# moabarar/nemar

Measured on AMD Instinct MI355X. Metric: train images/sec (256x256 A/B pairs), higher is better.
Workload: dtype f32

## Files before the change

include/nemar_hip.h:

```cpp
#ifndef NEMAR_HIP_H
#define NEMAR_HIP_H
#include <stddef.h>

#ifdef __cplusplus
extern "C" {
#endif

#define NEMAR_OK 0
#define NEMAR_EINVAL (-1)
#define NEMAR_ELAUNCH (-2)
#define NEMAR_EWORKSPACE (-3)

int nemar_version(void);
const char* nemar_last_error(void);

#define NEMAR_GRID_EXPLICIT 0
#define NEMAR_GRID_UNET 1
#define NEMAR_GRID_AFFINE 2
int nemar_grid_sample_fwd(const float* in, const float* grid_src, int grid_mode, float* out,
                          int N, int C, int H, int W, int Ho, int Wo, void* stream);
size_t nemar_grid_sample_bwd_workspace(int N, int C, int H, int W);
size_t nemar_grid_sample_bwd_zeroed_bytes(int N, int C, int H, int W);
int nemar_grid_sample_bwd(const float* in, const float* grid_src, int grid_mode, const float* gout,
                          float* gin, int accum_gin, float* ggrid, int accum_ggrid,
// ... 63 lines not shown
int nemar_conv2d_bwd_weight_ex(const float* x0, int C0, const float* x1, int C1, const float* gy, float* gw, float* gb, int N,
                               int H, int W, int K, int OH, int OW, int R, int S, int stride, int pad, int pad_mode,
                               void* workspace, size_t ws_bytes, void* stream, const nemar_conv_extras* extras);
int nemar_pack_plan_record(int plan);
int nemar_pack_plan_jobs(int plan);
size_t nemar_pack_plan_bytes(int plan);
int nemar_pack_plan_dirty(int plan);
int nemar_pack_plan_commit(int plan, void* device_buffer, size_t bytes, void* stream);
int nemar_pack_plan_run(int plan, void* stream);
int nemar_pack_plan_reset(int plan);
int nemar_last_route(void);
int nemar_config_epoch(void);
int nemar_set_max_words_lazy(int on);
int nemar_max_words_finalize(void* max_words, int samples, void* stream);
size_t nemar_conv2d_scratch(int N, int H, int W, int K, int C, int R, int S, int stride, int pad);
int nemar_absmax(const float* t, long long n, void* out_word, void* stream);
int nemar_absmax_samples(const float* t, int samples, long long per_sample, void* out_words, void* stream);
int nemar_kernel_timer(int enable);
int nemar_kernel_timer_read(double* total_ms, double* total_flop, int* launches);
size_t nemar_bias_grad_workspace(int N, int C, int HW);
int nemar_bias_grad(const float* g, float* gb, int N, int C, int HW, void* workspace, size_t ws_bytes, void* stream);

int nemar_instnorm_fwd(const float* x, const float* residual, float* y, float* stats, int planes, int HW,
                       float eps, int act, float slope, void* stream);
int nemar_instnorm_bwd(const float* x, const float* stats, const float* gy, float* gx, int planes, int HW,
                       int act, float slope, void* stream);
#define NEMAR_MAX_PARTIALS 2048
#define NEMAR_MAX_WORDS(samples) ((size_t)(samples) * (1 + NEMAR_MAX_PARTIALS))
int nemar_instnorm_fwd_max(const float* x, const float* residual, float* y, float* stats, int planes, int HW,
                           float eps, int act, float slope, void* max_words, int planes_per_sample, void* stream);
// ... 99 lines not shown
```

nemar_amd/_lib.py:

```python
import ctypes as C
import os

import torch

_HERE = os.path.dirname(os.path.abspath(__file__))
PRODUCT_PATH = os.path.join(_HERE, "lib", "libnemar_hip.so")
AB_PATH = os.path.join(_HERE, "lib", "libnemar_hip_ab.so")
DEFAULT_PATH = AB_PATH if (os.environ.get("NEMAR_AB_LIBRARY") == "1" or os.environ.get("NEMAR_TUNE")) else PRODUCT_PATH

_f = C.POINTER(C.c_float)
_vp = C.c_void_p
_i = C.c_int
_fl = C.c_float
_sz = C.c_size_t
_ll = C.c_longlong
_db = C.c_double
_u64 = C.c_ulonglong
_u32 = C.c_uint

SIGNATURES = {
    "nemar_version": (_i, []),
    "nemar_last_error": (C.c_char_p, []),
    "nemar_grid_sample_fwd": (_i, [_vp, _vp, _i, _vp, _i, _i, _i, _i, _i, _i, _vp]),
    "nemar_grid_sample_bwd_workspace": (_sz, [_i, _i, _i, _i]),
# ... 2 lines not shown
    "nemar_smoothness_workspace": (_sz, [_i, _i, _i]),
    "nemar_smoothness_fwd": (_i, [_vp, _vp, _i, _fl, _fl, _vp, _i, _vp, _sz, _i, _i, _i, _vp]),
    "nemar_smoothness_bwd": (_i, [_vp, _vp, _i, _fl, _vp, _fl, _vp, _i, _i, _i, _i, _vp]),
    "nemar_fold_penalty_workspace": (_sz, [_i, _i, _i]),
    "nemar_fold_penalty_fwd": (_i, [_vp, _fl, _fl, _vp, _i, _vp, _vp, _sz, _i, _i, _i, _vp]),
    "nemar_fold_penalty_bwd": (_i, [_vp, _fl, _vp, _fl, _vp, _i, _i, _i, _i, _vp]),
    "nemar_conv2d_fwd_workspace": (_sz, [_i] * 9),
    "nemar_conv2d_fwd": (_i, [_vp, _i, _vp, _i, _vp, _vp, _vp, _i, _i, _i, _i, _i, _i, _i, _i, _i, _i, _fl, _vp, _sz, _i, _vp]),
    "nemar_conv2d_bwd_data_workspace": (_sz, [_i] * 10),
    "nemar_conv2d_bwd_data": (_i, [_vp, _vp, _vp, _i, _fl, _vp, _i, _vp, _i, _i, _i, _i, _i, _i, _i, _i, _i, _i, _i,
                                   _i, _vp, _sz, _i, _vp]),
    "nemar_conv2d_bwd_weight_workspace": (_sz, [_i] * 11),
    "nemar_conv2d_bwd_weight": (_i, [_vp, _i, _vp, _i, _vp, _vp, _vp, _i, _i, _i, _i, _i, _i, _i, _i, _i, _i, _i, _vp, _sz,
                                     _vp]),
    "nemar_conv2d_scratch": (_sz, [_i] * 9),
    "nemar_conv2d_gy_planes_bytes": (_sz, [_i] * 10),
    "nemar_absmax": (_i, [_vp, _ll, _vp, _vp]),
    "nemar_absmax_samples": (_i, [_vp, _i, _ll, _vp, _vp]),
    "nemar_kernel_timer": (_i, [_i]),
    "nemar_kernel_timer_read": (_i, [C.POINTER(C.c_double), C.POINTER(C.c_double), C.POINTER(_i)]),
    "nemar_bias_grad_workspace": (_sz, [_i, _i, _i]),
    "nemar_bias_grad": (_i, [_vp, _vp, _i, _i, _i, _vp, _sz, _vp]),
    "nemar_last_route": (_i, []),
    "nemar_last_gy_planes": (_i, []),
    "nemar_config_epoch": (_i, []),
    "nemar_set_max_words_lazy": (_i, [_i]),
    "nemar_instnorm_fwd": (_i, [_vp, _vp, _vp, _vp, _i, _i, _fl, _i, _fl, _vp]),
    "nemar_instnorm_bwd": (_i, [_vp, _vp, _vp, _vp, _i, _i, _i, _fl, _vp]),
    "nemar_instnorm_fwd_max": (_i, [_vp, _vp, _vp, _vp, _i, _i, _fl, _i, _fl, _vp, _i, _vp]),
    "nemar_instnorm_fwd_planes": (_i, [_vp, _vp, _vp, _vp, _vp, _i, _i, _i, _i, _fl, _i, _fl, _fl, _u64, _u32, _vp, _vp, _vp, _vp, _vp]),
# ... 159 lines not shown
```

nemar_amd/csrc/conv.hip:

```cpp
#define NEMAR_CONV_HIP
#include "common.h"
#include "conv_exact.h"
#include "conv_call.h"
#include "conv_route.h"
#include "pack_plan.h"

#ifdef NEMAR_AB
extern int g_split16_ring3;
extern int g_split16_ksplit_cap;
extern int g_narrow_fwd4;
extern int g_wg_xreg;
extern int g_register_vec4;
extern int g_overlap_per_lane;
extern int g_histogram_per_lane;
void nemar_norm_planes_debug(int bits);
#endif

int nemar_narrow_fwd(const float* x, const float* w, const float* bias, float* y, int N, int C, int H, int W, int K, int R,
                     int pad, int border, int act, float slope, float* part, size_t part_floats, hipStream_t st);
int nemar_narrow_wgrad(const float* x, const float* gy, float* gw, int N, int C, int H, int W, int K, int R, int pad,
                       int border, float* part, hipStream_t st);
void nemar_wgrad2_launch(const float* x0, int C0, const float* x1, int C1, const float* gy, float* gw, float* gb, int N,
                         int H, int W, int K, int OH, int OW, int R, int S, int stride, int pad, int pad_mode,
                         int target_blocks, bool vec_ok, int dbg, float* part, hipStream_t st);
// ... 796 lines not shown
        if (gb) bias_grad_slabs(gy, gb, part ? part + P.bias_off : nullptr, N, K, OH * OW, st);
        what = "conv2d_bwd_weight (narrow)";
        break;
    case WgradPlan::S16G:
        nemar_s16g_wgrad(x0, C0, x1, C1, gy, gw, gb, N, H, W, K, OH, OW, R, stride, pad_mode, part, g_dbg, st);
        what = "conv2d_bwd_weight (16-bit pipe, in-kernel split)";
        break;
    case WgradPlan::SPLIT16:
        call.bias_rode = gb && call.bias_partials;
        nemar_split16_wgrad(x0, gy, gw, N, C0, H, W, K, R, pad_mode == BORDER_REFLECT ? 1 : 0, call.scratch, part, g_xcd_map,
                            R == 3 ? call.src2_planes : nullptr, (R == 3 && pad_mode == BORDER_REFLECT) ? call.x_planes : nullptr,
                            call.src_max, call.src2_max, call.bias_rode ? call.bias_partials : nullptr, gb, st);
        if (gb && !call.bias_rode) bias_grad_slabs(gy, gb, part + P.bias_off, N, K, OH * OW, st);
        what = "conv2d_bwd_weight (split-16)";
        break;
    case WgradPlan::WGRAD2:
        nemar_wgrad2_launch(x0, C0, x1, C1, gy, gw, gb, N, H, W, K, OH, OW, R, S, stride, pad, pad_mode, g_wgrad_blocks,
                            g_wgrad != 2, g_dbg, part, st);
        what = "conv2d_bwd_weight (wide)";
        break;
    case WgradPlan::WGRAD2_PADDED_GY: {
        float* gyp = part + P.gyp_off;
        const long long total = (long long)N * K * P.ohv * OW;
        hipLaunchKernelGGL(pad_planes_kernel, dim3(nemar_stream_grid(total, 256)), dim3(256), 0, st, gy, gyp, OH * OW, P.ohv * OW, total);
        nemar_wgrad2_launch(x0, C0, x1, C1, gyp, gw, gb, N, H, W, K, P.ohv, OW, R, S, stride, pad, pad_mode, g_wgrad_blocks,
                            g_wgrad != 2, g_dbg, part, st);
        what = "conv2d_bwd_weight (wide, padded gy)";
        break;
    }
    case WgradPlan::LEGACY: {
// ... 25 lines not shown
NEMAR_API int nemar_tune_ptr(void* p) { g_tl = (long long*)p; return NEMAR_OK; }

NEMAR_API int nemar_tune(int key, int value) {
    ++g_config_epoch;
    if (key == 0) { g_cfg128 = value; return NEMAR_OK; }
    if (key == 1) { g_lds_pad = value; return NEMAR_OK; }
    if (key == 2) { g_dbg = value; return NEMAR_OK; }
    if (key == 3) { g_narrow = value; return NEMAR_OK; }
    if (key == 4) { g_wgrad = value; return NEMAR_OK; }
    if (key == 6) { g_min_blocks = value > 0 ? value : 384; return NEMAR_OK; }
    if (key == 14) { g_deterministic = value != 0; return NEMAR_OK; }
    if (key == 8) { g_reflect_aux = value != 0; return NEMAR_OK; }
    if (key == 15) { g_xcd_map = value != 0; return NEMAR_OK; }
    if (key == 20) { g_split16 = value != 0; return NEMAR_OK; }
    if (key == 24) { g_s16g = value != 0; return NEMAR_OK; }
    if (key == 25) { g_s16g_min_mmac = value < 0 ? 0 : value; return NEMAR_OK; }
    if (key == 26) { g_s16g_wgrad_first = value != 0; return NEMAR_OK; }
    if (key == 27) { nemar_s16g_tune(0, value); return NEMAR_OK; }
    if (key == 29) { g_s16g_wgrad = value != 0; return NEMAR_OK; }
    if (key == 31) { nemar_norm_planes_debug(value); return NEMAR_OK; }
    if (key == 32) { g_split16_ring3 = value != 0; return NEMAR_OK; }
    if (key == 33) { g_k7 = value != 0; return NEMAR_OK; }
    if (key == 36) { g_split_act = value != 0; return NEMAR_OK; }
    if (key == 43) { g_fold_small = value != 0; return NEMAR_OK; }
    if (key == 37) { g_lds_claim = value; return NEMAR_OK; }
    if (key == 38) { g_wg_xreg = value != 0; return NEMAR_OK; }
    if (key == 39) { g_split16_ksplit_cap = value < 1 ? 1 : (value > 8 ? 8 : value); return NEMAR_OK; }
    if (key == 45) { g_overlap_per_lane = value != 0; return NEMAR_OK; }
    if (key == 46) { g_histogram_per_lane = value != 0; return NEMAR_OK; }
    if (key == 44) { g_register_vec4 = value != 0; return NEMAR_OK; }
// ... 20 lines not shown
}
#endif

static DgradPlan usual_dgrad(int N, int C, int H, int W, int K, int R, int S, int stride, int pad, int pad_mode) {
    DgradPlan P{};
    if (N <= 0 || C <= 0 || H <= 0 || W <= 0 || K <= 0 || R <= 0 || S <= 0 || stride < 1) return P;
    return plan_dgrad({N, C, 0, H, W, K, R, S, stride, pad, pad_mode}, ConvFacts::canonical());
}
static bool fusable(const DgradPlan& P) { return P.gy_planes_need != 0 && P.split16_ksplit == 1; }

NEMAR_API size_t nemar_conv2d_scratch(int N, int H, int W, int K, int C, int R, int S, int stride, int pad) {
    if (N <= 0 || H <= 0 || W <= 0 || K <= 0 || C <= 0) return 0;
    return plan_arena_bytes({N, C, 0, H, W, K, R, S, stride, pad, BORDER_ZERO});
}

NEMAR_API size_t nemar_conv2d_gy_planes_bytes(int N, int C, int H, int W, int K, int R, int S, int stride, int pad, int pad_mode) {
    return usual_dgrad(N, C, H, W, K, R, S, stride, pad, pad_mode).gy_planes_need;
}

NEMAR_API int nemar_conv2d_bwd_data_fusable(int N, int C, int H, int W, int K, int R, int S, int stride, int pad, int pad_mode) {
    return fusable(usual_dgrad(N, C, H, W, K, R, S, stride, pad, pad_mode)) ? 1 : 0;
}

NEMAR_API int nemar_conv2d_bwd_data_addend_ok(int N, int C, int H, int W, int K, int R, int S, int stride, int pad, int pad_mode) {
    const DgradPlan P = usual_dgrad(N, C, H, W, K, R, S, stride, pad, pad_mode);
    if (fusable(P)) return 1;
    if (pad_mode != BORDER_REFLECT || pad <= 0 || stride != 1 || pad >= H || pad >= W || R != S || R == 7) return 0;
    return (P.fold16 || P.fold) && plan_arena_bytes({N, C, 0, H, W, K, R, S, stride, pad, BORDER_ZERO}) == 0 ? 1 : 0;
}

// ... 128 lines not shown
```

nemar_amd/csrc/conv_route.h:

```cpp
#pragma once
#ifndef NEMAR_CONV_HIP
#error "conv_route.h holds conv.hip's own switches: include it from conv.hip only"
#endif
#include "common.h"
#include "conv_exact.h"
#include "conv_split16.h"
#include "conv_s16g.h"
#include "conv_k7.h"

bool nemar_narrow_eligible(int K, int C1, int R, int S, int stride, int N, int OH, int OW);
int nemar_narrow_wgrad_splits(int N, int C, int OH, int OW);
bool nemar_wgrad2_eligible(int K, int OH, int OW, bool gy_aligned16);
void nemar_wgrad2_plan(int K, int J, int P, int target_blocks, int* splits_out, int* pix_per_split_out);

using namespace nemar_exact;

namespace {

static NEMAR_SWITCH(int, g_split16, 1);
static NEMAR_SWITCH(long long, g_split16_min_mmac, 2000);
static NEMAR_SWITCH(int, g_split16_variant, 4);
static NEMAR_SWITCH(int, g_k7, 1);
static NEMAR_SWITCH(int, g_s16g, 1);
static NEMAR_SWITCH(long long, g_s16g_min_mmac, 30);
static NEMAR_SWITCH(int, g_s16g_wgrad, 1);
static NEMAR_SWITCH(int, g_s16g_wgrad_first, 0);
static NEMAR_SWITCH(int, g_s16g_fold, 1);
static NEMAR_SWITCH(int, g_split_act, 1);
static NEMAR_SWITCH(int, g_fold_small, 1);
static NEMAR_SWITCH(int, g_dual_gy, 1);
static NEMAR_SWITCH(int, g_reflect_aux, 1);
static NEMAR_SWITCH(int, g_deterministic, 1);
static NEMAR_SWITCH(int, g_ksplit, 1);
static NEMAR_SWITCH(int, g_narrow, 1);
static NEMAR_SWITCH(int, g_wgrad, 0);
static NEMAR_SWITCH(int, g_wgrad_blocks, 512);

// ... 308 lines not shown
        L.route = ROUTE_S16G; L.sub = DgradPlan::S16G;
        L.q.act = f.act; L.q.slope = f.slope;
    } else if (L.fold16 && f.gx0 && !f.gx1 && !f.bias && f.act == ACT_NONE) {
        L.route = ROUTE_S16G; L.sub = DgradPlan::S16G_FOLD;
    } else {
        L.route = ROUTE_EXACT; L.sub = DgradPlan::EXACT;
        L.narrow = g_narrow && stride == 1 && !L.fold && !f.bias && f.act == ACT_NONE && L.mskip == 0 && !f.gx1 && R - 1 - pad >= 0 &&
                   nemar_narrow_eligible(C, 0, R, S, 1, N, H, W);
        L.split = !L.narrow && L.ksplit > 1 && !f.bias && f.act == ACT_NONE && L.mskip == 0 &&
                  (L.fold ? (f.gx0 && !f.gx1) : (!f.gx1 || (f.gx0 && !L.ring)));
        L.aux_rows = !L.narrow && L.ring && g_reflect_aux && pad == 1 && R == 3 && S == 3 && H >= 4 && W >= 8;
    }
    return L;
}

void legacy_wgrad_plan(int K, int J, int P, int* splits_out, int* pix_per_split_out) {
    const bool wide = K > 32;
    const int BM = wide ? 128 : 32, BN = wide ? 128 : 256;
    const int mt = nemar_cdiv(K, BM), jt = nemar_cdiv(J, BN);
    int splits = nemar_cdiv(1024, mt * jt);
    const int max_splits = nemar_cdiv(P, WBK * 8);
    if (splits > max_splits) splits = max_splits;
    if (splits < 1) splits = 1;
    if (splits > 65535) splits = 65535;
    *pix_per_split_out = nemar_cdiv(nemar_cdiv(P, splits), WBK) * WBK;
    *splits_out = nemar_cdiv(P, *pix_per_split_out);
}
int padded_rows(int OH, int OW) {
    int ohv = OH;
    while ((ohv * OW) % 4) ++ohv;
    return ohv;
}
bool wgrad_pad_route(int K, int OH, int OW, int pad_mode) {
    return K > 4 && (OH * OW) % 4 != 0 && pad_mode == BORDER_ZERO && g_wgrad != 1;
}

struct WgradPlan {
    int route;
    enum Sub { K7, NARROW, S16G, SPLIT16, WGRAD2, WGRAD2_PADDED_GY, LEGACY } sub;
    size_t total, bias_off, gyp_off;
    int splits, pix_per_split, ohv;
};
WgradPlan plan_wgrad(const ConvShape& s, const ConvFacts& f) {
    WgradPlan P;
    const int N = s.N, C = s.C(), H = s.H, W = s.W, K = s.K, R = s.R, S = s.S, stride = s.stride, pad = s.pad, OH = s.OH(), OW = s.OW();
    const int J = C * R * S, Pix = N * OH * OW, ohv = padded_rows(OH, OW);
    const size_t slab = (size_t)K * J, bias_parts = (size_t)N * nemar_cdiv(OH * OW, BIAS_CHUNK) * K;
    int w2_splits, legacy_splits, pad_splits = 0, pps;
    nemar_wgrad2_plan(K, J, Pix, g_wgrad_blocks, &w2_splits, &pps);
    legacy_wgrad_plan(K, J, Pix, &legacy_splits, &P.pix_per_split);
    P.total = (size_t)(w2_splits > legacy_splits ? w2_splits : legacy_splits) * (slab + K);
    if ((OH * OW) % 4 != 0 && K > 4) {
        nemar_wgrad2_plan(K, J, N * ohv * OW, g_wgrad_blocks, &pad_splits, &pps);
        grow(P.total, (size_t)pad_splits * (slab + K) + 4 + (size_t)N * K * ohv * OW);
    }
    if (K <= 4) grow(P.total, (size_t)nemar_narrow_wgrad_splits(N, C, OH, OW) * slab + bias_parts);
    if (nemar_s16g_wgrad_eligible(N, C, 0, H, W, K, OH, OW, R, S, stride, pad, BORDER_ZERO))
        grow(P.total, (size_t)nemar_s16g_wgrad_slabs_max(N, C, K, OH, W, stride) * (slab + K));
    const bool k7 = nemar_k7_wgrad_eligible(N, C, H, W, K, R, S, stride, pad);
    if (k7) grow(P.total, nemar_k7_wgrad_floats(N, C, H, W, K) + bias_parts);
    const bool wide = wide_candidates(s).wgrad;
    if (wide) grow(P.total, (size_t)nemar_split16_wgrad_splits(N, C, H, W, K, R) * slab + bias_parts);
    const bool s16g_wg = g_s16g_wgrad && f.part && s16g_worth_it(s.macs()) &&
                         nemar_s16g_wgrad_eligible(N, s.C0, s.C1, H, W, K, OH, OW, R, S, stride, pad, s.pad_mode);
    const bool split16_wg = g_split16 && g_split16_variant == 4 && f.part && s.C1 == 0 && split16_worth_it(N, OH, OW, K, C, R, S) && wide &&
                            (R == 3 || s.pad_mode == BORDER_ZERO) && f.scratch_bytes &&
                            f.scratch_bytes >= nemar_split16_wgrad_scratch_bytes(N, C, H, W, K, R);
    P.bias_off = P.gyp_off = 0; P.splits = 0; P.ohv = ohv;
    if (g_k7 && f.part && s.C1 == 0 && k7) {
        P.route = ROUTE_K7; P.sub = WgradPlan::K7; P.bias_off = nemar_k7_wgrad_floats(N, C, H, W, K);
    } else if (nemar_narrow_eligible(K, s.C1, R, S, stride, N, OH, OW) && g_narrow) {
        P.route = ROUTE_NARROW; P.sub = WgradPlan::NARROW; P.bias_off = (size_t)nemar_narrow_wgrad_splits(N, s.C0, OH, OW) * slab;
    } else if (s16g_wg && (g_s16g_wgrad_first || !split16_wg)) {
        P.route = ROUTE_S16G; P.sub = WgradPlan::S16G;
    } else if (split16_wg) {
        P.route = ROUTE_SPLIT16; P.sub = WgradPlan::SPLIT16; P.bias_off = (size_t)nemar_split16_wgrad_splits(N, C, H, W, K, R) * slab;
    } else {
        P.route = ROUTE_EXACT;
        P.gyp_off = ((size_t)pad_splits * (slab + K) + 3) & ~(size_t)3;
        const bool padded_gy = f.part && wgrad_pad_route(K, OH, OW, s.pad_mode) && nemar_wgrad2_eligible(K, ohv, OW, f.part_aligned);
        if (g_wgrad != 1 && nemar_wgrad2_eligible(K, OH, OW, f.gy_aligned)) P.sub = WgradPlan::WGRAD2;
        else if (padded_gy) P.sub = WgradPlan::WGRAD2_PADDED_GY;
        else { P.sub = WgradPlan::LEGACY; P.splits = legacy_splits; P.bias_off = (size_t)legacy_splits * slab; }
    }
    return P;
}

size_t plan_arena_bytes(const ConvShape& s) {
    const int N = s.N, C = s.C(), H = s.H, W = s.W, K = s.K, R = s.R;
    if (!g_split16 || !split16_worth_it(N, H + 2 * s.pad - R + 1, W + 2 * s.pad - s.S + 1, K, C, R, s.S)) return 0;
    const WideCandidates c = wide_candidates(s);
    size_t b = c.fwd ? nemar_split16_scratch_total(N, H, W, K, C, H, W) : 0;
    if (c.dgrad) grow(b, nemar_split16_scratch_total(N, H, W, C, K, H, W));
    if (c.wgrad) grow(b, nemar_split16_wgrad_scratch_bytes(N, C, H, W, K, R));
    return b;
}

}
```

nemar_amd/csrc/conv_split16.h:

```cpp
#pragma once
#include <hip/hip_runtime.h>
#include <stddef.h>
#include "conv_call.h"

enum { SPLIT16_ZERO = 0, SPLIT16_REFLECT = 1, SPLIT16_DGRAD_REFLECT = 2 };

bool nemar_split16_eligible(int N, int H, int W, int M, int Cred, int R, int S, int stride, int pad, int mode, int variant);
size_t nemar_split16_scratch_bytes(int N, int Cred, int H, int W);
int nemar_split16_ksplit(int N, int H, int W, int M, int Cred);
size_t nemar_split16_scratch_total(int N, int H, int W, int M, int Cred, int OH, int OW);
size_t nemar_split16_pack_bytes(int M, int Cred, int KS);
void nemar_split16_pack(const float* w, void* packed, int K, int C, int KS, int dgrad, int variant, hipStream_t st);
struct Split16Done {
    bool dual_written;
    bool epilogue_fused;
};
Split16Done nemar_split16_conv(const float* src, const void* packed, const float* bias, float* dst, int N, int H, int W, int M, int Cred,
                               int KS, int src_pad, int Hs, int Ws_src, int OH, int OW, int mode, void* scratch, int xcd_map, int variant,
                               long long* tl, void* dual_g_out, MaxWords src_max, const void* ready_planes, int ready_kind,
                               const float* addend, void* out_max, hipStream_t st);

bool nemar_split16_wgrad_eligible(int N, int C, int H, int W, int K, int R, int S, int stride, int pad);
size_t nemar_split16_wgrad_scratch_bytes(int N, int C, int H, int W, int K, int KS);
int nemar_split16_wgrad_splits(int N, int C, int H, int W, int K, int KS);
#ifdef NEMAR_AB
void nemar_split16_wgrad_tune(int one_copy);
#endif
void nemar_sum_partials_pair(const float* part_a, long long stride_a, int splits_a, float* dst_a, long long n_a,
                             const float* part_b, long long stride_b, int splits_b, float* dst_b, long long n_b, bool accumulate, hipStream_t st);
void nemar_split16_wgrad(const float* x, const float* gy, float* gw, int N, int C, int H, int W, int K, int KS, int reflect,
                         void* scratch, float* part, int xcd_map, const void* g_planes, const void* x_planes, MaxWords x_max,
                         MaxWords gy_max, const float* bias_partials, float* gb, hipStream_t st);
size_t nemar_split16_wgrad_g_bytes(int N, int H, int W, int K, int KS);
void nemar_split16_dual_split(const float* gy, void* dplanes, void* gplanes, int N, int K, int H, int W, int mode, const unsigned* maxbits,
                              int mstride, hipStream_t st);
void nemar_sum_partials(const float* part, long long stride, int splits, float* dst, long long n, bool accumulate, hipStream_t st);
void nemar_sum_partials_two(const float* part, long long stride, int splits, float* d0, float* d1, int N, int C0, int C1, int HW, hipStream_t st);
void nemar_sum_partials_act(const float* part, long long stride, int splits, float* dst, long long n, int act, float slope, hipStream_t st);

void nemar_split16_absmax(const float* x, int samples, long long per, void* out, hipStream_t st);
const unsigned* nemar_split16_source_max(const float* src, int N, long long per, MaxWords hint, unsigned* own, int* stride, hipStream_t st);

void nemar_split16_timer(int on);
int nemar_split16_timer_read(double* total_ms, double* total_flop);
```

nemar_amd/csrc/conv_split16_wgrad.hip:

```cpp
#include "common.h"
#include "conv_split16.h"

namespace {

typedef float f32x16 __attribute__((ext_vector_type(16)));
typedef _Float16 f16x8 __attribute__((ext_vector_type(8)));
typedef unsigned u32x4 __attribute__((ext_vector_type(4)));

__device__ __forceinline__ float pow2_scale(unsigned maxbits) {
    const int e = (int)((maxbits >> 23) & 255u);
    if (e == 0 || e == 255) return 1.f;
    const int se = 127 + 11 - (e - 127);
    if (se < 1 || se > 254) return 1.f;
    return __builtin_bit_cast(float, (unsigned)se << 23);
}
__device__ __forceinline__ unsigned short f16_rn(float v) {
    const _Float16 h = (_Float16)v;
    return __builtin_bit_cast(unsigned short, h);
}
__device__ __forceinline__ void split2_f16(float v, unsigned short& h, unsigned short& l) {
    h = f16_rn(v);
    const float r = v - (float)__builtin_bit_cast(_Float16, h);
    l = f16_rn(r);
}
// ... 73 lines not shown
#pragma unroll
        for (int e = 0; e < 8; ++e) {
            const int xs = q * 8 + e - 1;
            v[e] = tile[cc][min(max(reflect ? mirror(xs, W) : xs, 0), W - 1)];
        }
#pragma unroll
        for (int e = 0; e < 8; ++e) {
            const int xp = q * 8 + e;
            const bool ok = xp < W + 2 && (reflect || (unsigned)(xp - 1) < (unsigned)W);
            split2_f16(ok ? v[e] : 0.f, h[e], l[e]);
        }
        const size_t t = (((size_t)n * CBLK + cblk) * FX + (size_t)yp * CPR + q) * 64 + cc;
        out[t] = pack8(h);
        out[total + t] = pack8(l);
    }
}

template <int TW>
__global__ __launch_bounds__(256) void split_dual_kernel(const float* __restrict__ gy, u32x4* __restrict__ dpl, u32x4* __restrict__ gpl,
                                                         int N, int K, int H, int W, int Hg, int CPR, int reflect, long long dtotal,
                                                         long long gtotal, const unsigned* maxbits, int mstride) {
    __shared__ float tile[64][TW + 1];
    const int Hp = H + 4, Ws = W + 4, KBLK = K >> 6, CG = K >> 3, F = Hg * CPR;
    const int prow = blockIdx.x % Hp, kblk = (blockIdx.x / Hp) % KBLK, n = blockIdx.x / (Hp * KBLK);
    const float scale = pow2_scale(maxbits[n * mstride]);
    const bool img = prow >= 1 && prow <= H;
    int ya = 0, yb = -1;
    bool any = img;
    if (img) ya = prow - 1;
    else if (reflect && prow == H + 2) { ya = 0; yb = 2; any = true; }
// ... 46 lines not shown
    const u32x4* G;
    const u32x4* X;
    float* part;
    int N, H, W, C, K;
    int CPR, F, FX, RB, spi;
    int KBLK, CBLK;
    long long gplane16, xplane16;
    const unsigned* gmax;
    const unsigned* xmax;
    int gstride, xstride;
    int xcd;
};

template <int KS, bool ONEG, bool XREG = false>
__global__ __launch_bounds__(256) void wgrad_split16_kernel(WgParams p) {
    static_assert(!XREG || (KS == 3 && ONEG), "XREG: instantiated and measured for the 3x3 one-copy form only");

    constexpr int GC = ONEG ? 1 : KS;
    constexpr int RING = 4, NCOL = 4 * GC + 4 * KS, NCP = NCOL / 4;
    constexpr int STAGE16 = NCOL * 64;
    constexpr int NMF = 3 * KS * KS, NSL = 2 * GC + 2 * KS + NCP;
    constexpr int NPV = KS / 2;
#ifdef NEMAR_HOST_EMULATION
    __shared__ __attribute__((aligned(16))) u32x4 smem[RING * STAGE16];
#else
    extern __shared__ __attribute__((aligned(16))) u32x4 smem[];
#endif
    const int tid = threadIdx.x, wid = __builtin_amdgcn_readfirstlane(tid >> 6), lane = tid & 63;
    const int tiles = p.KBLK * p.CBLK;
    int t = blockIdx.x;
    if (p.xcd) t = (t & 7) * ((int)gridDim.x >> 3) + (t >> 3);
// ... 280 lines not shown
    p.KBLK = KBLK; p.CBLK = CBLK;
    p.gplane16 = gtotal; p.xplane16 = xtotal;
    p.gmax = gmax; p.xmax = xmax; p.gstride = gstride; p.xstride = xstride;
    const int splits = N * p.spi, grid = splits * KBLK * CBLK;
    p.xcd = (xcd_map && grid % 8 == 0 && (grid / 8) % (KBLK * CBLK) == 0) ? 1 : 0;
    NEMAR_AB_ONLY(if (KS == 3 && oneg && !g_wg_xreg) wg_launch<3, true, false>(grid, p, st); else)
    if (KS == 3 && oneg) wg_launch<3, true, true>(grid, p, st);
    else if (oneg) wg_launch<4, true>(grid, p, st);
#ifdef NEMAR_AB
    else if (KS == 3) wg_launch<3, false>(grid, p, st);
    else wg_launch<4, false>(grid, p, st);
#endif
    nemar_sum_partials_pair(part, (long long)K * C * KS * KS, splits, gw, (long long)K * C * KS * KS, bias_partials, K, N,
                            bias_partials ? gb : nullptr, K, true, st);
}
```

nemar_amd/ops.py:

```python
import ctypes
import os
import weakref

import numpy as np

import torch
from torch.autograd import Function
from torch.autograd.function import once_differentiable

from . import _lib

L = _lib.load()



class _SizeQueries:

    def __init__(self, lib):
        self._lib, self._memo = lib, {}

    def __getattr__(self, name):
        fn = getattr(self._lib, name)
        memo = self._memo

# ... 185 lines not shown

def _conv_scratch(N, H, W, K, C, R, S, stride, pad, device):
    key = (N, H, W, K, C, R, S, stride, pad)
    need = _scratch_need.get(key)
    if need is None:
        need = _scratch_need[key] = L.conv2d_scratch(N, H, W, K, C, R, S, stride, pad)
    if not need:
        return None
    akey = (device, _lane[0])
    buf = _arena.get(akey)
    if buf is None or buf.numel() * 4 < need:
        _retire(buf)
        buf = torch.empty(int(need) // 4 + 64, dtype=torch.float32, device=device)
        _arena[akey] = buf
    return buf


_garena = {}
_garena_next = {}
_gplanes_need = {}
GY_RING = int(os.environ.get("NEMAR_GY_RING", "4"))
_GY_HANDOVER = os.environ.get("NEMAR_GY_HANDOVER", "1") == "1"


def _gy_planes(N, C, H, W, K, R, S, stride, pad, pad_mode, device):
    if _side_on[0] and not _GY_HANDOVER:
        return None, None
    key = (N, C, H, W, K, R, S, stride, pad, pad_mode)
    need = _gplanes_need.get(key)
    if need is None:
# ... 145 lines not shown
def _reset_plans():
    _plan_gen[0] += 1
    for o in list(_plan_owners):
        L.pack_plan_reset(o._plan)


def invalidate_packed_weights():
    _param_epoch.n += 1
    _reset_plans()


def tune(key, value):
    L.tune(key, value)
    Q._memo.clear()
    _scratch_need.clear()
    _gplanes_need.clear()
    _fusable.clear()
    _xplanes_need.clear()
    invalidate_packed_weights()


class _PackEntry:
    __slots__ = ('buf', 'token', 'ref', 'plan_gen')

    def __init__(self, buf, token, ref):
        self.buf, self.token, self.ref, self.plan_gen = buf, token, ref, -1


class _record:
    __slots__ = ('plan',)
# ... 78 lines not shown
        OW = (W + 2 * pad - S) // stride + 1
        y = torch.empty((N, K, OH, OW), dtype=torch.float32, device=x.device)
        wsb = Q.conv2d_fwd_workspace(N, H, W, K, C, R, S, stride, pad)
        ws, hit, plan = _packed(weight, ('fwd', stride, pad, N, H, W), wsb)
        arena = _conv_scratch(N, H, W, K, C, R, S, stride, pad, x.device) if x2 is None else None
        tag = 'igemm_fwd_resblock' if (K == 256 and C == 256 and R == 3 and pad_mode == PAD_REFLECT) else None
        with (_span(tag) if tag else contextlib.nullcontext()):
            xmax = ready = None
            if arena is not None:
                ready = _planes_of(x) if (pad_mode == PAD_REFLECT and R == 3 and S == 3 and stride == 1 and pad == 1) else None
                xmax = ready[1] if ready is not None else _absmax_word(x)
            with _record(plan):
                L.conv2d_fwd_ex(_p(x), C0, _p(x2), C1, _p(w), _p(b), _p(y), N, H, W, K, R, S, stride, pad, pad_mode, act,
                                slope, _p(ws), wsb, hit, _stream(), _extras(arena, xmax, None, ready[0] if ready is not None else None))
        ctx.xmax = xmax
        xp = _xplanes_of(x) if ready is not None else None
        ctx.xplanes = xp[0] if (xp is not None and xp[1] is ready[1]) else None
        ctx.grad_from = int(getattr(x, '_nemar_grad_from', 0)) if x2 is None else 0
        ctx.save_for_backward(x, x2, w, y if act != ACT_NONE else None)
        ctx.weight, ctx.bias = weight, bias
        _note_use(weight)
        if bias is not None:
            _note_use(bias)
        ctx.cfg = (stride, pad, pad_mode, act, slope)
        if with_skip:
            return y, x.view_as(x)
        return y

    @staticmethod
    @once_differentiable
# ... 4 lines not shown
        if gy is None:
            return (ctx.gskip,) + (None,) * 10
        gy = _c(gy)
        N, C0, H, W = x.shape
        C1 = 0 if x2 is None else x2.shape[1]
        K, C, R, S = w.shape
        OH, OW = gy.shape[2:]
        st = _stream()
        if act != ACT_NONE:
            g = torch.empty_like(gy)
            L.act_bwd(_p(gy), _p(y), _p(g), gy.numel(), act, slope, st)
        else:
            g = gy
        need_x, need_x2, need_w, need_b = ctx.needs_input_grad[0], ctx.needs_input_grad[1], \
            ctx.needs_input_grad[2], ctx.needs_input_grad[3]
        gmax = _absmax_word(g) if ctx.xmax is not None else None
        return _Conv2d._backward_body(ctx, x, x2, w, g, N, C0, C1, H, W, K, C, R, S, OH, OW, stride, pad, pad_mode, st,
                                      need_x, need_x2, need_w, need_b, gmax)

    @staticmethod
    def _backward_body(ctx, x, x2, w, g, N, C0, C1, H, W, K, C, R, S, OH, OW, stride, pad, pad_mode, st, need_x, need_x2, need_w,
                       need_b, gmax):
        gx = gx2 = gpl = gslot = None
        if need_x or need_x2:
            gx = torch.empty_like(x) if need_x else None
            gx2 = torch.empty_like(x2) if (need_x2 and x2 is not None) else None
            if x2 is not None and gx2 is None:
                gx2 = torch.empty_like(x2)
            wsb = Q.conv2d_bwd_data_workspace(N, C, H, W, K, R, S, stride, pad, pad_mode)
            if pad_mode == PAD_REFLECT and pad > 0 and x2 is not None:
                raise NotImplementedError("reflect-padded conv over a concatenated input has no data-gradient kernel")
# ... 36 lines not shown
            if _use and _side_on[0]:
                _side_touched.add(id(gwbuf))
                if gbbuf is not None:
                    _side_touched.add(id(gbbuf))
            else:
                _main_lane_grad(gwbuf, g.device)
                if gbbuf is not None:
                    _main_lane_grad(gbbuf, g.device)
            rbw = K == 256 and C == 256 and R == 3 and pad_mode == PAD_REFLECT
            xpl = getattr(ctx, 'xplanes', None)
            with (_on_side(g.device, x, x2, g, gmax, ctx.xmax, gpl, xpl) if _use else contextlib.nullcontext()), \
                    (_span('wgrad_resblock') if rbw else contextlib.nullcontext()):
                gb = _grad_buffer(ctx.bias) if want_b else None
                wsb = Q.conv2d_bwd_weight_workspace(N, C, H, W, K, OH, OW, R, S, stride, pad)
                arena = _conv_scratch(N, H, W, K, C, R, S, stride, pad, g.device)
                L.conv2d_bwd_weight_ex(_p(x), C0, _p(x2), C1, _p(g), _p(gwbuf), _p(gb), N, H, W, K, OH, OW,
                                       R, S, stride, pad, pad_mode, _p(_workspace(wsb, g.device)), wsb, _stream(),
                                       _extras(arena, ctx.xmax, gmax, planes=xpl, src2_planes=gpl))
                if gslot is not None and _side_on[0]:
                    ev = torch.cuda.Event()
                    ev.record(torch.cuda.current_stream(g.device))
                    gslot[1] = ev
                grad_ready(ctx.weight)
                if want_b:
                    grad_ready(ctx.bias)
        elif want_b:
            gbbuf = _grad_buffer(ctx.bias)
            _main_lane_grad(gbbuf, g.device)
            _bias_grad(g, gbbuf, N, K, OH * OW, st)
            grad_ready(ctx.bias)
# ... 1270 lines not shown
```

Before: 283.2.

## Route stride-2 4x4 conv weight gradients through space-to-depth split-16 kernel

Adds a space-to-depth path for 4x4 stride-2 pad-1 convolutions. The input is recast as a 2x2 stride-1 conv over 4C channels, so the existing split-16 fp16-pair matrix wgrad kernel can handle it. A new x-splitting kernel and a partial-sum kernel scatter results back into the 4x4 weight layout, and a dedicated scratch arena is sized from Python. The aim is to replace a slower generic wgrad route for downsampling convs, at the cost of extra split and reduce passes, more scratch memory, and extra absmax plumbing in backward.

```diff
diff --git a/include/nemar_hip.h b/include/nemar_hip.h
--- a/include/nemar_hip.h
+++ b/include/nemar_hip.h
@@ -101,6 +101,7 @@
 int nemar_set_max_words_lazy(int on);
 int nemar_max_words_finalize(void* max_words, int samples, void* stream);
 size_t nemar_conv2d_scratch(int N, int H, int W, int K, int C, int R, int S, int stride, int pad);
+size_t nemar_conv2d_bwd_weight_scratch(int N, int C, int H, int W, int K, int OH, int OW, int R, int S, int stride, int pad);
 int nemar_absmax(const float* t, long long n, void* out_word, void* stream);
 int nemar_absmax_samples(const float* t, int samples, long long per_sample, void* out_words, void* stream);
 int nemar_kernel_timer(int enable);
diff --git a/nemar_amd/_lib.py b/nemar_amd/_lib.py
--- a/nemar_amd/_lib.py
+++ b/nemar_amd/_lib.py
@@ -40,6 +40,7 @@
     "nemar_conv2d_bwd_weight": (_i, [_vp, _i, _vp, _i, _vp, _vp, _vp, _i, _i, _i, _i, _i, _i, _i, _i, _i, _i, _i, _vp, _sz,
                                      _vp]),
     "nemar_conv2d_scratch": (_sz, [_i] * 9),
+    "nemar_conv2d_bwd_weight_scratch": (_sz, [_i] * 11),
     "nemar_conv2d_gy_planes_bytes": (_sz, [_i] * 10),
     "nemar_absmax": (_i, [_vp, _ll, _vp, _vp]),
     "nemar_absmax_samples": (_i, [_vp, _i, _ll, _vp, _vp]),
diff --git a/nemar_amd/csrc/conv.hip b/nemar_amd/csrc/conv.hip
--- a/nemar_amd/csrc/conv.hip
+++ b/nemar_amd/csrc/conv.hip
@@ -834,6 +834,11 @@
         if (gb && !call.bias_rode) bias_grad_slabs(gy, gb, part + P.bias_off, N, K, OH * OW, st);
         what = "conv2d_bwd_weight (split-16)";
         break;
+    case WgradPlan::SPLIT16_S2D:
+        nemar_split16_wgrad_s2d(x0, gy, gw, N, C0, H, W, K, call.scratch, part, g_xcd_map, call.src_max, call.src2_max, st);
+        if (gb) bias_grad_slabs(gy, gb, part + P.bias_off, N, K, OH * OW, st);
+        what = "conv2d_bwd_weight (split-16, space-to-depth)";
+        break;
     case WgradPlan::WGRAD2:
         nemar_wgrad2_launch(x0, C0, x1, C1, gy, gw, gb, N, H, W, K, OH, OW, R, S, stride, pad, pad_mode, g_wgrad_blocks,
                             g_wgrad != 2, g_dbg, part, st);
@@ -889,6 +894,7 @@
     if (key == 15) { g_xcd_map = value != 0; return NEMAR_OK; }
     if (key == 20) { g_split16 = value != 0; return NEMAR_OK; }
     if (key == 24) { g_s16g = value != 0; return NEMAR_OK; }
+    if (key == 47) { g_wgrad_s2d = value != 0; return NEMAR_OK; }
     if (key == 25) { g_s16g_min_mmac = value < 0 ? 0 : value; return NEMAR_OK; }
     if (key == 26) { g_s16g_wgrad_first = value != 0; return NEMAR_OK; }
     if (key == 27) { nemar_s16g_tune(0, value); return NEMAR_OK; }
@@ -939,6 +945,11 @@
     return plan_arena_bytes({N, C, 0, H, W, K, R, S, stride, pad, BORDER_ZERO});
 }
 
+NEMAR_API size_t nemar_conv2d_bwd_weight_scratch(int N, int C, int H, int W, int K, int OH, int OW, int R, int S, int stride, int pad) {
+    if (N <= 0 || C <= 0 || H <= 0 || W <= 0 || K <= 0 || OH <= 0 || OW <= 0) return 0;
+    return plan_wgrad_arena_bytes({N, C, 0, H, W, K, R, S, stride, pad, BORDER_ZERO, OH, OW});
+}
+
 NEMAR_API size_t nemar_conv2d_gy_planes_bytes(int N, int C, int H, int W, int K, int R, int S, int stride, int pad, int pad_mode) {
     return usual_dgrad(N, C, H, W, K, R, S, stride, pad, pad_mode).gy_planes_need;
 }
diff --git a/nemar_amd/csrc/conv_route.h b/nemar_amd/csrc/conv_route.h
--- a/nemar_amd/csrc/conv_route.h
+++ b/nemar_amd/csrc/conv_route.h
@@ -21,6 +21,7 @@
 static NEMAR_SWITCH(long long, g_split16_min_mmac, 2000);
 static NEMAR_SWITCH(int, g_split16_variant, 4);
 static NEMAR_SWITCH(int, g_k7, 1);
+static NEMAR_SWITCH(int, g_wgrad_s2d, 1);
 static NEMAR_SWITCH(int, g_s16g, 1);
 static NEMAR_SWITCH(long long, g_s16g_min_mmac, 30);
 static NEMAR_SWITCH(int, g_s16g_wgrad, 1);
@@ -359,6 +360,12 @@
     return L;
 }
 
+bool wgrad_s2d_candidate(const ConvShape& s) {
+    return s.OH() == s.H / 2 && s.OW() == s.W / 2 && nemar_split16_wgrad_s2d_eligible(s.N, s.C(), s.H, s.W, s.K, s.R, s.S, s.stride, s.pad);
+}
+bool wgrad_s2d_on(const ConvShape& s) {
+    return g_split16 && g_split16_variant == 4 && g_wgrad_s2d && split16_worth_it(s.N, s.OH(), s.OW(), s.K, s.C(), s.R, s.S);
+}
 void legacy_wgrad_plan(int K, int J, int P, int* splits_out, int* pix_per_split_out) {
     const bool wide = K > 32;
     const int BM = wide ? 128 : 32, BN = wide ? 128 : 256;
@@ -382,7 +389,7 @@
 
 struct WgradPlan {
     int route;
-    enum Sub { K7, NARROW, S16G, SPLIT16, WGRAD2, WGRAD2_PADDED_GY, LEGACY } sub;
+    enum Sub { K7, NARROW, S16G, SPLIT16, SPLIT16_S2D, WGRAD2, WGRAD2_PADDED_GY, LEGACY } sub;
     size_t total, bias_off, gyp_off;
     int splits, pix_per_split, ohv;
 };
@@ -406,6 +413,10 @@
     if (k7) grow(P.total, nemar_k7_wgrad_floats(N, C, H, W, K) + bias_parts);
     const bool wide = wide_candidates(s).wgrad;
     if (wide) grow(P.total, (size_t)nemar_split16_wgrad_splits(N, C, H, W, K, R) * slab + bias_parts);
+    const bool s2d = wgrad_s2d_candidate(s);
+    if (s2d) grow(P.total, (size_t)nemar_split16_wgrad_s2d_splits(N, C, H, W, K) * slab + bias_parts);
+    const bool s2d_wg = s2d && wgrad_s2d_on(s) && f.part && s.C1 == 0 && s.pad_mode == BORDER_ZERO && f.scratch_bytes &&
+                        f.scratch_bytes >= nemar_split16_wgrad_s2d_scratch_bytes(N, C, H, W, K);
     const bool s16g_wg = g_s16g_wgrad && f.part && s16g_worth_it(s.macs()) &&
                          nemar_s16g_wgrad_eligible(N, s.C0, s.C1, H, W, K, OH, OW, R, S, stride, pad, s.pad_mode);
     const bool split16_wg = g_split16 && g_split16_variant == 4 && f.part && s.C1 == 0 && split16_worth_it(N, OH, OW, K, C, R, S) && wide &&
@@ -416,6 +427,8 @@
         P.route = ROUTE_K7; P.sub = WgradPlan::K7; P.bias_off = nemar_k7_wgrad_floats(N, C, H, W, K);
     } else if (nemar_narrow_eligible(K, s.C1, R, S, stride, N, OH, OW) && g_narrow) {
         P.route = ROUTE_NARROW; P.sub = WgradPlan::NARROW; P.bias_off = (size_t)nemar_narrow_wgrad_splits(N, s.C0, OH, OW) * slab;
+    } else if (s2d_wg) {
+        P.route = ROUTE_SPLIT16; P.sub = WgradPlan::SPLIT16_S2D; P.bias_off = (size_t)nemar_split16_wgrad_s2d_splits(N, C, H, W, K) * slab;
     } else if (s16g_wg && (g_s16g_wgrad_first || !split16_wg)) {
         P.route = ROUTE_S16G; P.sub = WgradPlan::S16G;
     } else if (split16_wg) {
@@ -441,4 +454,10 @@
     return b;
 }
 
-}
+
+size_t plan_wgrad_arena_bytes(const ConvShape& s) {
+    if (!wgrad_s2d_candidate(s) || !wgrad_s2d_on(s)) return 0;
+    return nemar_split16_wgrad_s2d_scratch_bytes(s.N, s.C(), s.H, s.W, s.K);
+}
+
+}
diff --git a/nemar_amd/csrc/conv_split16.h b/nemar_amd/csrc/conv_split16.h
--- a/nemar_amd/csrc/conv_split16.h
+++ b/nemar_amd/csrc/conv_split16.h
@@ -31,6 +31,11 @@
 void nemar_split16_wgrad(const float* x, const float* gy, float* gw, int N, int C, int H, int W, int K, int KS, int reflect,
                          void* scratch, float* part, int xcd_map, const void* g_planes, const void* x_planes, MaxWords x_max,
                          MaxWords gy_max, const float* bias_partials, float* gb, hipStream_t st);
+bool nemar_split16_wgrad_s2d_eligible(int N, int C, int H, int W, int K, int R, int S, int stride, int pad);
+size_t nemar_split16_wgrad_s2d_scratch_bytes(int N, int C, int H, int W, int K);
+int nemar_split16_wgrad_s2d_splits(int N, int C, int H, int W, int K);
+void nemar_split16_wgrad_s2d(const float* x, const float* gy, float* gw, int N, int C, int H, int W, int K, void* scratch, float* part,
+                             int xcd_map, MaxWords x_max, MaxWords gy_max, hipStream_t st);
 size_t nemar_split16_wgrad_g_bytes(int N, int H, int W, int K, int KS);
 void nemar_split16_dual_split(const float* gy, void* dplanes, void* gplanes, int N, int K, int H, int W, int mode, const unsigned* maxbits,
                               int mstride, hipStream_t st);
diff --git a/nemar_amd/csrc/conv_split16_wgrad.hip b/nemar_amd/csrc/conv_split16_wgrad.hip
--- a/nemar_amd/csrc/conv_split16_wgrad.hip
+++ b/nemar_amd/csrc/conv_split16_wgrad.hip
@@ -111,6 +111,62 @@
         out[t] = pack8(h);
         out[total + t] = pack8(l);
     }
+}
+
+template <int TW>
+__global__ __launch_bounds__(256) void split_wgrad_x_s2d_kernel(const float* __restrict__ x, u32x4* __restrict__ out, int N, int C, int H, int W,
+                                                                int Hp, int CPR, long long total, const unsigned* maxbits, int mstride) {
+    __shared__ float tile[32][TW + 2];
+    const int CBLK = C >> 4, FX = Hp * CPR;
+    const int yy = blockIdx.x % Hp, cblk = (blockIdx.x / Hp) % CBLK, n = blockIdx.x / (Hp * CBLK);
+    const float scale = pow2_scale(maxbits[n * mstride]);
+    for (int i = threadIdx.x; i < 32 * W; i += 256) {
+        const int j = i / W, xs = i - j * W;
+        const int t = cblk * 32 + j, a = t / C, c = t - a * C;
+        const int ys = 2 * yy + a - 1;
+        const bool rowok = (unsigned)ys < (unsigned)H;
+        const float v = x[(((size_t)n * C + c) * H + (rowok ? ys : 0)) * W + xs];
+        tile[j][xs] = rowok ? v * scale : 0.f;
+    }
+    __syncthreads();
+    const int cc = threadIdx.x & 63, j = cc >> 1, b = cc & 1;
+    for (int q = threadIdx.x >> 6; q < CPR; q += 4) {
+        unsigned short h[8], l[8];
+        float v[8];
+#pragma unroll
+        for (int e = 0; e < 8; ++e) v[e] = tile[j][min(max(2 * (q * 8 + e) + b - 1, 0), W - 1)];
+#pragma unroll
+        for (int e = 0; e < 8; ++e) {
+            const int xs = 2 * (q * 8 + e) + b - 1;
+            split2_f16((unsigned)xs < (unsigned)W ? v[e] : 0.f, h[e], l[e]);
+        }
+        const size_t t = (((size_t)n * CBLK + cblk) * FX + (size_t)yy * CPR + q) * 64 + cc;
+        out[t] = pack8(h);
+        out[total + t] = pack8(l);
+    }
+}
+
+__global__ __launch_bounds__(256) void sum_partials_s2d_kernel(const float* __restrict__ part, long long stride, int splits, float* __restrict__ gw,
+                                                               int C, long long cols) {
+    typedef float f32x4 __attribute__((ext_vector_type(4)));
+    const long long i = (long long)blockIdx.x * 256 + threadIdx.x;
+    if (i >= cols) return;
+    const int C4 = 4 * C, k = (int)(i / C4), cp = (int)(i - (long long)k * C4), b = cp & 1, t = cp >> 1, a = t / C, c = t - a * C;
+    f32x4 acc = {0.f, 0.f, 0.f, 0.f};
+    for (int s0 = 0; s0 < splits; s0 += 8) {
+        f32x4 v[8];
+#pragma unroll
+        for (int e = 0; e < 8; ++e)
+            v[e] = *reinterpret_cast<const f32x4*>(part + (long long)min(s0 + e, splits - 1) * stride + 4 * i);
+#pragma unroll
+        for (int e = 0; e < 8; ++e)
+            if (s0 + e < splits) acc += v[e];
+    }
+    float* const o = gw + ((size_t)k * C + c) * 16 + 4 * a + b;
+    o[0] += acc[0];
+    o[2] += acc[1];
+    o[8] += acc[2];
+    o[10] += acc[3];
 }
 
 template <int TW>
@@ -187,7 +243,7 @@
 
 template <int KS, bool ONEG, bool XREG = false>
 __global__ __launch_bounds__(256) void wgrad_split16_kernel(WgParams p) {
-    static_assert(!XREG || (KS == 3 && ONEG), "XREG: instantiated and measured for the 3x3 one-copy form only");
+    static_assert(!XREG || ((KS == 3 || KS == 2) && ONEG), "XREG: instantiated and measured for the one-copy 3x3 and 2x2 (space-to-depth) forms only");
 
     constexpr int GC = ONEG ? 1 : KS;
     constexpr int RING = 4, NCOL = 4 * GC + 4 * KS, NCP = NCOL / 4;
@@ -498,3 +554,61 @@
     nemar_sum_partials_pair(part, (long long)K * C * KS * KS, splits, gw, (long long)K * C * KS * KS, bias_partials, K, N,
                             bias_partials ? gb : nullptr, K, true, st);
 }
+
+static int s2d_cpr(int W) { return (W / 2 + 1 + 7) / 8; }
+
+bool nemar_split16_wgrad_s2d_eligible(int N, int C, int H, int W, int K, int R, int S, int stride, int pad) {
+    if (R != 4 || S != 4 || stride != 2 || pad != 1) return false;
+    if (H % 2 || W % 2 || H < 8 || W < 8 || W > SPLIT_MAXW || N > 256) return false;
+    if (C % 16 || K % 64 || C < 32 || K < 128) return false;
+    const int CPR = s2d_cpr(W), Hg = g_rows(H / 2 - 1, 2);
+    if (rows_per_split(N, Hg, CPR, (K / 64) * (C / 16)) == 0) return false;
+    if ((long long)N * (4 * C > K ? 4 * C : K) * (Hg + 1) * CPR * 64 >= (1ll << 31)) return false;
+    return true;
+}
+
+size_t nemar_split16_wgrad_s2d_scratch_bytes(int N, int C, int H, int W, int K) {
+    const int CPR = s2d_cpr(W), Hg = g_rows(H / 2 - 1, 2);
+    return ((size_t)2 * N * K * Hg * CPR + (size_t)2 * N * 4 * C * (Hg + 1) * CPR) * 16 + 16384;
+}
+
+int nemar_split16_wgrad_s2d_splits(int N, int C, int H, int W, int K) {
+    const int CPR = s2d_cpr(W), Hg = g_rows(H / 2 - 1, 2);
+    const int rb = rows_per_split(N, Hg, CPR, (K / 64) * (C / 16));
+    return rb ? N * (Hg / rb) : 0;
+}
+
+void nemar_split16_wgrad_s2d(const float* x, const float* gy, float* gw, int N, int C, int H, int W, int K, void* scratch, float* part,
+                             int xcd_map, MaxWords x_max, MaxWords gy_max, hipStream_t st) {
+    const int OH = H / 2, OW = W / 2, CV = 4 * C, CPR = s2d_cpr(W), KBLK = K / 64, CBLK = CV / 64;
+    const int Hg = g_rows(OH - 1, 2), Hx = Hg + 1;
+    const long long gtotal = (long long)N * K * Hg * CPR, xtotal = (long long)N * CV * Hx * CPR;
+    u32x4* const G = (u32x4*)scratch;
+    u32x4* const X = G + 2 * gtotal;
+    unsigned* const mw = (unsigned*)((char*)scratch + nemar_split16_wgrad_s2d_scratch_bytes(N, C, H, W, K) - 2048);
+    int gstride = 0, xstride = 0;
+    const unsigned* const gmax = nemar_split16_source_max(gy, N, (long long)K * OH * OW, gy_max, mw, &gstride, st);
+    const unsigned* const xmax = nemar_split16_source_max(x, N, (long long)C * H * W, x_max, mw + 256, &xstride, st);
+#define WG_SPLIT_G(TW_)                                                                                                            \
+    hipLaunchKernelGGL((split_wgrad_g_kernel<TW_, 1>), dim3(N * KBLK * Hg), dim3(256), 0, st, gy, G, N, K, OH, OW, Hg, CPR, gtotal, gmax, gstride);
+#define WG_SPLIT_X(TW_)                                                                                                            \
+    hipLaunchKernelGGL((split_wgrad_x_s2d_kernel<TW_>), dim3(N * CBLK * Hx), dim3(256), 0, st, x, X, N, C, H, W, Hx, CPR, xtotal, xmax, xstride);
+    if (OW <= 64) { WG_SPLIT_G(64) } else { WG_SPLIT_G(128) }
+    if (W <= 64) { WG_SPLIT_X(64) } else if (W <= 128) { WG_SPLIT_X(128) } else { WG_SPLIT_X(256) }
+#undef WG_SPLIT_G
+#undef WG_SPLIT_X
+    WgParams p;
+    p.G = G; p.X = X; p.part = part;
+    p.N = N; p.H = OH - 1; p.W = OW - 1; p.C = CV; p.K = K;
+    p.CPR = CPR; p.F = Hg * CPR; p.FX = Hx * CPR;
+    p.RB = rows_per_split(N, Hg, CPR, KBLK * CBLK);
+    p.spi = Hg / p.RB;
+    p.KBLK = KBLK; p.CBLK = CBLK;
+    p.gplane16 = gtotal; p.xplane16 = xtotal;
+    p.gmax = gmax; p.xmax = xmax; p.gstride = gstride; p.xstride = xstride;
+    const int splits = N * p.spi, grid = splits * KBLK * CBLK;
+    p.xcd = (xcd_map && grid % 8 == 0 && (grid / 8) % (KBLK * CBLK) == 0) ? 1 : 0;
+    wg_launch<2, true, true>(grid, p, st);
+    const long long cols = (long long)K * CV;
+    hipLaunchKernelGGL(sum_partials_s2d_kernel, dim3((unsigned)((cols + 255) / 256)), dim3(256), 0, st, part, cols * 4, splits, gw, C, cols);
+}
diff --git a/nemar_amd/ops.py b/nemar_amd/ops.py
--- a/nemar_amd/ops.py
+++ b/nemar_amd/ops.py
@@ -223,6 +223,36 @@
         buf = torch.empty(int(need) // 4 + 64, dtype=torch.float32, device=device)
         _arena[akey] = buf
     return buf
+
+
+_wgrad_scratch_need = {}
+
+
+def _wgrad_arena_bytes(N, C, H, W, K, OH, OW, R, S, stride, pad):
+    key = (N, C, H, W, K, OH, OW, R, S, stride, pad)
+    need = _wgrad_scratch_need.get(key)
+    if need is None:
+        need = _wgrad_scratch_need[key] = L.conv2d_bwd_weight_scratch(N, C, H, W, K, OH, OW, R, S, stride, pad)
+    return need
+
+
+def _wgrad_scratch(N, C, H, W, K, OH, OW, R, S, stride, pad, device):
+    need = _wgrad_arena_bytes(N, C, H, W, K, OH, OW, R, S, stride, pad)
+    if not need:
+        return None
+    akey = (device, _lane[0])
+    buf = _arena.get(akey)
+    if buf is None or buf.numel() * 4 < need:
+        _retire(buf)
+        buf = torch.empty(int(need) // 4 + 64, dtype=torch.float32, device=device)
+        _arena[akey] = buf
+    return buf
+
+
+def _published_max(t):
+    if getattr(t, '_nemar_absmax', None) is None and getattr(t, '_nemar_absmax_lazy', None) is None:
+        return None
+    return _absmax_word(t)
 
 
 _garena = {}
@@ -398,6 +428,7 @@
     L.tune(key, value)
     Q._memo.clear()
     _scratch_need.clear()
+    _wgrad_scratch_need.clear()
     _gplanes_need.clear()
     _fusable.clear()
     _xplanes_need.clear()
@@ -506,6 +537,7 @@
                 L.conv2d_fwd_ex(_p(x), C0, _p(x2), C1, _p(w), _p(b), _p(y), N, H, W, K, R, S, stride, pad, pad_mode, act,
                                 slope, _p(ws), wsb, hit, _stream(), _extras(arena, xmax, None, ready[0] if ready is not None else None))
         ctx.xmax = xmax
+        ctx.wgrad_wide = arena is None and x2 is None and _wgrad_arena_bytes(N, C, H, W, K, OH, OW, R, S, stride, pad) > 0
         xp = _xplanes_of(x) if ready is not None else None
         ctx.xplanes = xp[0] if (xp is not None and xp[1] is ready[1]) else None
         ctx.grad_from = int(getattr(x, '_nemar_grad_from', 0)) if x2 is None else 0
@@ -540,7 +572,11 @@
             g = gy
         need_x, need_x2, need_w, need_b = ctx.needs_input_grad[0], ctx.needs_input_grad[1], \
             ctx.needs_input_grad[2], ctx.needs_input_grad[3]
-        gmax = _absmax_word(g) if ctx.xmax is not None else None
+        if getattr(ctx, 'wgrad_wide', False):
+            gmax = _published_max(g) if need_w else None
+            ctx.xmax = _published_max(x) if need_w else None
+        else:
+            gmax = _absmax_word(g) if ctx.xmax is not None else None
         return _Conv2d._backward_body(ctx, x, x2, w, g, N, C0, C1, H, W, K, C, R, S, OH, OW, stride, pad, pad_mode, st,
                                       need_x, need_x2, need_w, need_b, gmax)
 
@@ -607,6 +643,8 @@
                 gb = _grad_buffer(ctx.bias) if want_b else None
                 wsb = Q.conv2d_bwd_weight_workspace(N, C, H, W, K, OH, OW, R, S, stride, pad)
                 arena = _conv_scratch(N, H, W, K, C, R, S, stride, pad, g.device)
+                if arena is None and x2 is None:
+                    arena = _wgrad_scratch(N, C, H, W, K, OH, OW, R, S, stride, pad, g.device)
                 L.conv2d_bwd_weight_ex(_p(x), C0, _p(x2), C1, _p(g), _p(gwbuf), _p(gb), N, H, W, K, OH, OW,
                                        R, S, stride, pad, pad_mode, _p(_workspace(wsb, g.device)), wsb, _stream(),
                                        _extras(arena, ctx.xmax, gmax, planes=xpl, src2_planes=gpl))
```

Result: no change. 285.8, median of 6 (+0.9%).
